# SrikarK-code/clip-dplm

Hardware: NVIDIA B200
Metric: contrastive_fwd_bwd_pairs_per_sec (higher is better)
Workload: dtype bf16

## Files before the change

clip-dplm_b200/csrc/clipnce_api.cu:

```cuda
#include <cuda.h>
#include <cuda_bf16.h>
#include <cuda_runtime.h>

#include <cmath>
#include <cstdarg>
#include <cstdio>
#include <cstdlib>
#include <cstring>
#include <mutex>
#include <set>
#include <string>
#include <utility>

#include "../../include/clipnce.h"
#include "kernels_aux.cuh"
#include "kernels_head.cuh"
#include "kernels_link.cuh"
#include "kernels_pair.cuh"
#include "kernels_pair2.cuh"
#include "kernels_simt.cuh"
#include "kernels_tc.cuh"

namespace {

thread_local std::string g_err;

int fail(int code, const char* fmt, ...) {
  char buf[512];
  va_list ap;
  va_start(ap, fmt);
  vsnprintf(buf, sizeof buf, fmt, ap);
  va_end(ap);
  g_err = buf;
  return code;
}

#define CUDA_TRY(expr)                                                                              \
  do {                                                                                              \
    cudaError_t e_ = (expr);                                                                        \
    if (e_ != cudaSuccess) return fail(CLIPNCE_ECUDA, "%s: %s", #expr, cudaGetErrorString(e_));     \
  } while (0)

// ... 927 lines not shown
  const dim3 grid((unsigned)pl.n_blk, (unsigned)n_members);
  const int64_t slab_elems = 2 * V * d;
#define FINISH_G(TI, TO)                                                                                                  \
  aux::finish_rows_group<__nv_bfloat16, TI, TO><<<grid, 256, smem, st>>>(slabs, pl.bwd_n_split, slab_elems, fg,          \
                                                                        (const __nv_bfloat16*)stack, (const TI*)stack_orig, \
                                                                        rinv, di, (TO*)d_stack, ds_part, sq_part)
  if (in_dtype == CLIPNCE_BF16 && out_dtype == CLIPNCE_BF16) FINISH_G(__nv_bfloat16, __nv_bfloat16);
  else if (in_dtype == CLIPNCE_BF16) FINISH_G(__nv_bfloat16, float);
  else if (out_dtype == CLIPNCE_BF16) FINISH_G(float, __nv_bfloat16);
  else FINISH_G(float, float);
#undef FINISH_G
  CUDA_TRY(cudaGetLastError());
  if (d_scale_sum || grad_sumsq) {
    aux::reduce_group_scalars<<<1 + n_members, 256, 0, st>>>(ds_part, sq_part, n_members, pl.n_blk, d_scale_sum, grad_sumsq);
    CUDA_TRY(cudaGetLastError());
  }
  return 0;
}

}

namespace {
struct Bwd2Plan {
  int P, Q, n_rb, n_seg, seg_steps, n_items, n_rounds, n_steps, n_half, depth, stages_a, stages_b, stages_c, smem;
  size_t off_flags, off_ring, off_dxh, off_dyh, off_part, bytes;
};

bool bwd2_device_ok() {
  if (env_int("CLIPNCE_NO_BWD2", 0) != 0) return false;
  if (allow_smem(pair2::bwd2_kernel<false>, pair::SMEM_LIMIT) || allow_smem(pair2::bwd2_kernel<true>, pair::SMEM_LIMIT)) {
    cudaGetLastError();
    return false;
  }
  static const bool ok = [] {
    cudaLaunchConfig_t cfg;
    memset(&cfg, 0, sizeof cfg);
    cfg.gridDim = dim3(2 * pair_slots());
    cfg.blockDim = dim3(pair2::THREADS);
    cfg.dynamicSmemBytes = pair::SMEM_LIMIT;
    int n = 0, n2 = 0;
    if (cudaOccupancyMaxActiveClusters(&n, pair2::bwd2_kernel<false>, &cfg) != cudaSuccess ||
        cudaOccupancyMaxActiveClusters(&n2, pair2::bwd2_kernel<true>, &cfg) != cudaSuccess) {
      cudaGetLastError();
      return false;
    }
    return n >= pair_slots() && n2 >= pair_slots();
  }();
  return ok;
}

bool bwd2_plan(int64_t n_rows, int64_t n_cols, int64_t d, int dtype, float scale, int flags, int world, Bwd2Plan* pl) {
  const int fam = tc_family(dtype, d, scale, flags);
  if (!((fam == 1 || fam == 2) && pair_eligible(d)) || (flags & CLIPNCE_FLAG_UNBOUNDED)) return false;
  if (world == 1 || world < 0 || world > pair2::MAX_WORLD) return false;
  if (world == 0 ? n_rows != n_cols : n_rows * world != n_cols) return false;
  const int64_t min_n = env_int("CLIPNCE_BWD2_MIN_N", 12288);
  if (n_rows % 128 != 0 || n_cols % 256 != 0 || n_rows * n_cols < min_n * min_n || n_cols > (1ll << 22)) return false;
  if (world >= 2 && (n_cols / world) % 256 != 0) return false;
  const int slots = pair_slots();
  if (slots < 8) return false;
  pl->n_rb = (int)(n_rows / 128);
  pl->n_steps = (int)(n_cols / 256);
  pl->n_half = (int)ceil_div(d, 256);
  const int forced_p = (int)env_int("CLIPNCE_BWD2_P", 0);
  const int forced_seg = (int)env_int("CLIPNCE_BWD2_SEG", 0);
  constexpr double r = 1.0;
  double best_t = 1e300;
  int best_p = 0, best_seg = 0;
  for (int n_seg = 1; n_seg <= 8; n_seg *= 2) {
    int ns = world >= 2 ? world : n_seg;
    if (world == 0 && forced_seg >= 1) ns = forced_seg;
    if (pl->n_steps % ns != 0) continue;
    const int seg_steps = pl->n_steps / ns;
    if (seg_steps < 8 && ns > 1 && world == 0 && forced_seg < 1) continue;
    const int64_t n_items = (int64_t)pl->n_rb * ns;
    const double slab_steps = (double)(ns - 1) * (double)n_rows * (double)d * 8.0 / 3e12 / 3.9e-6;
    const bool force = forced_p >= 1 && forced_p <= slots - 1;
    for (int Pe = force ? forced_p : slots / 2; Pe <= (force ? forced_p : slots - 2); ++Pe) {
      const int Q = slots - Pe;
      const double tp = (double)ceil_div(n_items, Pe) * ((double)seg_steps + 1.0);
      const double tc_ = (double)n_items * (double)seg_steps / ((double)Q * 2.0 * r);
      const double t = ((tp > tc_ ? tp : tc_) + slab_steps) * (world == 0 && ns > 1 ? 1.08 : 1.0);
      if (t < best_t - 1e-9) { best_t = t; best_p = Pe; best_seg = ns; }
    }
    if (world >= 2 || forced_seg >= 1) break;
  }
  if (best_p == 0) return false;
  pl->P = best_p;
  pl->Q = slots - best_p;
  pl->n_seg = best_seg;
  pl->seg_steps = pl->n_steps / best_seg;
  pl->n_items = pl->n_rb * best_seg;
  pl->n_rounds = (int)ceil_div(pl->n_items, pl->P);
  pl->depth = pair2::RING_DEPTH;
  const int nkc = (int)(d / 64);
  const int total = (pair::SMEM_LIMIT - pair2::producer_smem(nkc, 0)) / pair::STAGE_BYTES;
  if (total < 4) return false;
  auto cap = [](int v) { return v > pair2::MAXS ? pair2::MAXS : v; };
  pl->stages_b = cap(total / 2);
  pl->stages_a = cap(total - total / 2);
  pl->stages_c = cap((pair::SMEM_LIMIT - pair2::consumer_smem(0)) / pair2::C_STAGE);
  const int ps = pair2::producer_smem(nkc, pl->stages_a + pl->stages_b), cs = pair2::consumer_smem(pl->stages_c);
  pl->smem = ps > cs ? ps : cs;
  size_t off = 0;
  auto region = [&](size_t bytes) { const size_t o = off; off = (size_t)round_up((int64_t)(off + bytes), 256); return o; };
  pl->off_flags = region(sizeof(uint32_t) * 2 * (size_t)pl->n_rounds * (size_t)pl->seg_steps);
  pl->off_ring = region((size_t)pl->depth * (size_t)pl->P * 128 * 256 * 2);
  pl->off_dxh = region(sizeof(float) * (size_t)pl->n_seg * (size_t)n_rows * (size_t)d);
  pl->off_dyh = region(sizeof(float) * (size_t)n_cols * (size_t)d);
  pl->off_part = region(sizeof(float) * (size_t)ceil_div(n_rows > n_cols ? n_rows : n_cols, 8));
  pl->bytes = off;
  return true;
}

int launch_finish(const float* parts, int n_split, int64_t slab_elems, const void* xc, const void* xo, int in_dtype,
                  const float* rinv, const float* grad_scale, int64_t n, int64_t d, void* dx, int out_dtype, float* ds_part,
                  cudaStream_t st) {
  const unsigned grid = (unsigned)ceil_div(n, 8);
  const size_t smem = sizeof(float) * 8 * (size_t)d;
  const int di = (int)d;
#define FINISH3(TI, TO)                                                                                                \
  aux::finish_rows_v4<__nv_bfloat16, TI, TO><<<grid, 256, smem, st>>>(parts, n_split, slab_elems, (const __nv_bfloat16*)xc, \
                                                                      (const TI*)xo, rinv, grad_scale, n, di, (TO*)dx, ds_part)
  if (in_dtype == CLIPNCE_BF16 && out_dtype == CLIPNCE_BF16) FINISH3(__nv_bfloat16, __nv_bfloat16);
  else if (in_dtype == CLIPNCE_BF16) FINISH3(__nv_bfloat16, float);
  else if (out_dtype == CLIPNCE_BF16) FINISH3(float, __nv_bfloat16);
  else FINISH3(float, float);
#undef FINISH3
  CUDA_TRY(cudaGetLastError());
  return 0;
// ... 1 lines not shown

int bwd2_launch(const Bwd2Plan& pl, const void* x, const void* y, const float* rinv_x, const float* rinv_y, int64_t n_rows,
                int64_t n_cols, int64_t d, int64_t diag_offset, float scale, const float* scale_dev, const float* row_m,
                const float* row_w, const float* col_m, const float* col_w, float diag_w, char* ws, float* const* dy_peer,
                int world, cudaStream_t st) {
  uint32_t* flags_dev = reinterpret_cast<uint32_t*>(ws + pl.off_flags);
  const size_t n_flags = (size_t)pl.n_rounds * (size_t)pl.seg_steps;
  CUDA_TRY(cudaMemsetAsync(flags_dev, 0, sizeof(uint32_t) * 2 * n_flags, st));
  pair2::Params p;
  memset(&p, 0, sizeof p);
  p.n_rows = (int)n_rows; p.n_cols = (int)n_cols; p.d = (int)d;
  p.nkc = (int)(d / 64); p.nq2 = (int)ceil_div(d, 256); p.n_half = pl.n_half;
  p.nsbuf = p.nq2 <= 2 ? 2 : 1;
  p.n_rb = pl.n_rb; p.n_seg = pl.n_seg; p.seg_steps = pl.seg_steps; p.n_items = pl.n_items; p.n_rounds = pl.n_rounds;
  p.P = pl.P; p.Q = pl.Q; p.depth = pl.depth;
  p.stages_a = pl.stages_a; p.stages_b = pl.stages_b; p.stages_c = pl.stages_c;
  p.diag_offset = diag_offset; p.scale = scale; p.scale_dev = scale_dev; p.diag_w = diag_w;
  p.rinv_x = rinv_x; p.rinv_y = rinv_y; p.row_m = row_m; p.row_w = row_w; p.col_m = col_m; p.col_w = col_w;
  p.dx = reinterpret_cast<float*>(ws + pl.off_dxh);
  p.dy = reinterpret_cast<float*>(ws + pl.off_dyh);
  p.world = world;
  for (int s = 0; s < world; ++s) p.dy_peer[s] = dy_peer[s];
  p.ready = flags_dev; p.done = flags_dev + n_flags;
  CUtensorMap tx, ty, tyg, tg;
  int rc;
  if ((rc = make_tmap(&tx, x, d, n_rows, d, pair2::ROWS))) return rc;
  if ((rc = make_tmap(&ty, y, d, n_cols, d, 128))) return rc;
  if ((rc = make_tmap(&tyg, y, d, n_cols, d, 64))) return rc;
  if ((rc = make_tmap(&tg, ws + pl.off_ring, 256, (int64_t)pl.depth * pl.P * 128, 256, 64))) return rc;
  auto kern = tc_family(CLIPNCE_BF16, d, scale, 0) == 2 ? pair2::bwd2_kernel<true> : pair2::bwd2_kernel<false>;
  if ((rc = allow_smem(kern, pair::SMEM_LIMIT))) return rc;
  kern<<<2 * (pl.P + pl.Q), pair2::THREADS, pl.smem, st>>>(tx, ty, tyg, tg, p);
  CUDA_TRY(cudaGetLastError());
  return 0;
}
}

extern "C" {

int clipnce_backward_both_workspace_bytes(int64_t n_rows, int64_t n_cols, int64_t d, int dtype, float scale, int flags,
                                          int world, size_t* out) {
  if (!out) return fail(CLIPNCE_EINVAL, "backward_both_workspace_bytes: null pointer");
  Bwd2Plan pl;
  *out = (n_rows >= 1 && n_cols >= 1 && d >= 1 && bwd2_plan(n_rows, n_cols, d, dtype, scale, flags, world, &pl) &&
          check_device_sm100() == 0 && bwd2_device_ok()) ? pl.bytes : 0;
  return 0;
}

int clipnce_backward_both_dx(const void* x, const void* y, const float* rinv_x, const float* rinv_y, int64_t n,
                             int64_t d, float scale, const float* scale_dev, const float* row_m, const float* row_w,
                             const float* col_m, const float* col_w, float diag_w, int dtype, int flags,
                             const void* x_orig, const void* y_orig, int in_dtype, const float* grad_scale, void* dx,
                             void* dy, int out_dtype, float* d_scale_sum, void* workspace, size_t workspace_bytes,
                             void* stream) {
  if (!x || !y || !rinv_x || !rinv_y || !row_m || !row_w || !col_m || !col_w || !x_orig || !y_orig || !dx || !dy || !workspace)
    return fail(CLIPNCE_EINVAL, "backward_both_dx: null pointer");
  if ((in_dtype != CLIPNCE_BF16 && in_dtype != CLIPNCE_F32) || (out_dtype != CLIPNCE_BF16 && out_dtype != CLIPNCE_F32))
    return fail(CLIPNCE_EINVAL, "backward_both_dx: bad dtype");
  if (in_dtype == dtype && (x_orig != x || y_orig != y))
    return fail(CLIPNCE_EINVAL, "backward_both_dx: x_orig / y_orig of the compute type must be x / y themselves");
  if (!aligned16(x) || !aligned16(y) || !aligned16(workspace)) return fail(CLIPNCE_EINVAL, "backward_both_dx: operands must be 16-byte aligned");
  int rc = check_device_sm100();
  if (rc) return rc;
  Bwd2Plan pl;
  if (!bwd2_plan(n, n, d, dtype, scale, flags, 0, &pl) || !bwd2_device_ok())
    return fail(CLIPNCE_EUNSUPPORTED, "backward_both_dx: shape not served (see clipnce_backward_both_workspace_bytes)");
  if (workspace_bytes < pl.bytes) return fail(CLIPNCE_EWORKSPACE, "backward_both_dx: workspace %zu < %zu", workspace_bytes, pl.bytes);
  cudaStream_t st = as_stream(stream);
  char* ws = reinterpret_cast<char*>(workspace);
  if ((rc = bwd2_launch(pl, x, y, rinv_x, rinv_y, n, n, d, 0, scale, scale_dev, row_m, row_w, col_m, col_w, diag_w, ws, nullptr,
                        0, st)))
    return rc;
  float* ds_part = reinterpret_cast<float*>(ws + pl.off_part);
  if ((rc = launch_finish(reinterpret_cast<float*>(ws + pl.off_dxh), pl.n_seg, n * d, x, x_orig, in_dtype, rinv_x, grad_scale, n, d,
                          dx, out_dtype, d_scale_sum ? ds_part : nullptr, st)))
    return rc;
  if ((rc = launch_finish(reinterpret_cast<float*>(ws + pl.off_dyh), 1, n * d, y, y_orig, in_dtype, rinv_y, grad_scale, n, d, dy,
                          out_dtype, nullptr, st)))
    return rc;
  if (d_scale_sum) {
    aux::reduce_scalar_partials_par<<<1, 256, 0, st>>>(ds_part, (int)ceil_div(n, 8), 1.f, d_scale_sum);
    CUDA_TRY(cudaGetLastError());
  }
  return 0;
}

int clipnce_backward_both_sharded(const void* x, const void* y, const float* rinv_x, const float* rinv_y, int64_t n_rows,
                                  int64_t n_cols, int64_t d, int64_t diag_offset, float scale, const float* scale_dev,
                                  const float* row_m, const float* row_w, const float* col_m, const float* col_w,
                                  float diag_w, int dtype, int flags, const void* x_orig, int in_dtype,
                                  const float* grad_scale, void* dx, int out_dtype, float* d_scale_sum,
                                  void* const* peer_base, int world, int rank, int64_t slots_offset, void* workspace,
                                  size_t workspace_bytes, void* stream) {
  if (!x || !y || !rinv_x || !rinv_y || !row_m || !row_w || !col_m || !col_w || !x_orig || !workspace || !peer_base)
    return fail(CLIPNCE_EINVAL, "backward_both_sharded: null pointer");
  if ((in_dtype != CLIPNCE_BF16 && in_dtype != CLIPNCE_F32) || (out_dtype != CLIPNCE_BF16 && out_dtype != CLIPNCE_F32))
    return fail(CLIPNCE_EINVAL, "backward_both_sharded: bad dtype");
  if (in_dtype == dtype && x_orig != x) return fail(CLIPNCE_EINVAL, "backward_both_sharded: x_orig of the compute type must be x itself");
  if (!aligned16(x) || !aligned16(y) || !aligned16(workspace)) return fail(CLIPNCE_EINVAL, "backward_both_sharded: operands must be 16-byte aligned");
  if (world < 2 || world > pair2::MAX_WORLD || rank < 0 || rank >= world || slots_offset < 0 || slots_offset % 16 != 0)
    return fail(CLIPNCE_EINVAL, "backward_both_sharded: bad world / rank / slots_offset");
  if (diag_offset != (int64_t)rank * n_rows) return fail(CLIPNCE_EINVAL, "backward_both_sharded: diag_offset must be rank * n_rows");
  int rc = check_device_sm100();
  if (rc) return rc;
  Bwd2Plan pl;
  if (!bwd2_plan(n_rows, n_cols, d, dtype, scale, flags, world, &pl) || !bwd2_device_ok())
    return fail(CLIPNCE_EUNSUPPORTED, "backward_both_sharded: shape not served (see clipnce_backward_both_workspace_bytes)");
  if (workspace_bytes < pl.bytes) return fail(CLIPNCE_EWORKSPACE, "backward_both_sharded: workspace %zu < %zu", workspace_bytes, pl.bytes);
  cudaStream_t st = as_stream(stream);
  char* ws = reinterpret_cast<char*>(workspace);
  float* dy_peer[pair2::MAX_WORLD];
  for (int s = 0; s < world; ++s) {
    if (!peer_base[s] || !aligned16(peer_base[s])) return fail(CLIPNCE_EINVAL, "backward_both_sharded: peer buffer %d is null or unaligned", s);
    dy_peer[s] = reinterpret_cast<float*>(reinterpret_cast<char*>(peer_base[s]) + slots_offset) + (size_t)rank * (size_t)n_rows * (size_t)d;
  }
  if ((rc = bwd2_launch(pl, x, y, rinv_x, rinv_y, n_rows, n_cols, d, diag_offset, scale, scale_dev, row_m, row_w, col_m, col_w,
                        diag_w, ws, dy_peer, world, st)))
    return rc;
  if (!dx) return 0;
  float* ds_part = reinterpret_cast<float*>(ws + pl.off_part);
  if ((rc = launch_finish(reinterpret_cast<float*>(ws + pl.off_dxh), pl.n_seg, n_rows * d, x, x_orig, in_dtype, rinv_x, grad_scale,
                          n_rows, d, dx, out_dtype, d_scale_sum ? ds_part : nullptr, st)))
    return rc;
  if (d_scale_sum) {
    aux::reduce_scalar_partials_par<<<1, 256, 0, st>>>(ds_part, (int)ceil_div(n_rows, 8), 1.f, d_scale_sum);
    CUDA_TRY(cudaGetLastError());
  }
  return 0;
}
// ... 355 lines not shown
```

clip-dplm_b200/csrc/kernels_pair2.cuh:

```cuda
#pragma once
#include "kernels_pair.cuh"

namespace pair2 {

using pair::LOG2E;
using pair::STAGE_BYTES;
using pair::STEP_J;
using pair::TMEM_COLS;

constexpr int THREADS = 416;
constexpr int STORE_WARP = 12;
constexpr int EPI_WARPS = 8;
constexpr int ROWS = 64;
constexpr int X_CHUNK = ROWS * 128;
constexpr int G_BYTES = 4 * 8192;
constexpr int SMALL = 10240;
constexpr int C_STAGE = 32768;
constexpr int MAXS = 6;
constexpr int RING_DEPTH = 16;
constexpr int MAX_WORLD = 16;

constexpr int B_FULL_A = 0, B_EMPTY_A = MAXS, B_FULL_B = 2 * MAXS, B_EMPTY_B = 3 * MAXS, B_XFULL = 4 * MAXS,
              B_XEMPTY = B_XFULL + 1, B_SFULL = B_XEMPTY + 1, B_SEMPTY = B_SFULL + 2, B_GFULL = B_SEMPTY + 2,
              B_GEMPTY = B_GFULL + 4, B_ACCFULL = B_GEMPTY + 4, B_ACCEMPTY = B_ACCFULL + 2, B_GSFULL = B_ACCEMPTY + 2,
// ... 2 lines not shown

struct Params {
  int n_rows, n_cols, d;
  int nsbuf;
  int nkc, nq2, n_half;
  int n_rb, n_seg, seg_steps, n_items, n_rounds;
  int P, Q, depth;
  int stages_a, stages_b, stages_c;
  long long diag_offset;
  float scale, diag_w;
  const float* scale_dev;
  const float* rinv_x;
  const float* rinv_y;
  const float* row_m;
  const float* row_w;
  const float* col_m;
  const float* col_w;
  float* dx;
  float* dy;
  float* dy_peer[MAX_WORLD];
  int world;
  uint32_t* ready;
  uint32_t* done;
};

__host__ __device__ constexpr int producer_smem(int nkc, int stages) {
  return nkc * X_CHUNK + G_BYTES + stages * STAGE_BYTES + SMALL;
}
constexpr int FLUSH_BYTES = EPI_WARPS * 4096;
__host__ __device__ constexpr int consumer_smem(int stages) { return stages * C_STAGE + FLUSH_BYTES + SMALL; }
__device__ __forceinline__ float4 ld_shared_v4(uint32_t addr) {
  float4 v;
  asm volatile("ld.shared.v4.f32 {%0, %1, %2, %3}, [%4];" : "=f"(v.x), "=f"(v.y), "=f"(v.z), "=f"(v.w) : "r"(addr) : "memory");
  return v;
}

__device__ __forceinline__ void publish(uint32_t* flag) {
  ptx::fence_proxy_async_all();
  ptx::red_release_gpu_add(flag, 1u);
}

struct Sub {
  int seg, p_lo, p_hi, rb_lo;
  bool first, last;
};
__device__ __forceinline__ int round_items(const Params& p, int r) { return min(p.P, p.n_items - r * p.P); }
// ... 557 lines not shown
```

Measured before the change: 4.394 million.

## Add three-role backward kernel splitting producer, dX partner, and dY consumer

Introduces a new bwd3 kernel in which separate CTA pairs handle the logits/gradient producer, the dX accumulation partner, and the dY consumer, with 256-row blocks per item. It becomes the default for d up to 512. The planner is reworked to split SMs among the three roles, and the co-residency check is generalised per kernel and smem size. The intent is to balance tensor-core work across more specialized roles and to free producer shared memory for deeper pipelines. This adds a large new kernel and more inter-CTA flag synchronisation.

```diff
diff --git a/clip-dplm_b200/csrc/clipnce_api.cu b/clip-dplm_b200/csrc/clipnce_api.cu
--- a/clip-dplm_b200/csrc/clipnce_api.cu
+++ b/clip-dplm_b200/csrc/clipnce_api.cu
@@ -10,6 +10,7 @@
 #include <mutex>
 #include <set>
 #include <string>
+#include <tuple>
 #include <utility>
 
 #include "../../include/clipnce.h"
@@ -18,6 +19,7 @@
 #include "kernels_link.cuh"
 #include "kernels_pair.cuh"
 #include "kernels_pair2.cuh"
+#include "kernels_pair3.cuh"
 #include "kernels_simt.cuh"
 #include "kernels_tc.cuh"
 
@@ -991,31 +993,47 @@
 
 namespace {
 struct Bwd2Plan {
+  int roles;
+  int fam;
   int P, Q, n_rb, n_seg, seg_steps, n_items, n_rounds, n_steps, n_half, depth, stages_a, stages_b, stages_c, smem;
   size_t off_flags, off_ring, off_dxh, off_dyh, off_part, bytes;
 };
 
-bool bwd2_device_ok() {
-  if (env_int("CLIPNCE_NO_BWD2", 0) != 0) return false;
-  if (allow_smem(pair2::bwd2_kernel<false>, pair::SMEM_LIMIT) || allow_smem(pair2::bwd2_kernel<true>, pair::SMEM_LIMIT)) {
+std::set<std::tuple<const void*, int, int>> g_coresident;
+
+template <typename Kernel>
+bool coresident(Kernel* kern, int smem) {
+  int dev = 0;
+  if (allow_smem(kern, pair::SMEM_LIMIT) || cudaGetDevice(&dev) != cudaSuccess) {
     cudaGetLastError();
     return false;
   }
-  static const bool ok = [] {
-    cudaLaunchConfig_t cfg;
-    memset(&cfg, 0, sizeof cfg);
-    cfg.gridDim = dim3(2 * pair_slots());
-    cfg.blockDim = dim3(pair2::THREADS);
-    cfg.dynamicSmemBytes = pair::SMEM_LIMIT;
-    int n = 0, n2 = 0;
-    if (cudaOccupancyMaxActiveClusters(&n, pair2::bwd2_kernel<false>, &cfg) != cudaSuccess ||
-        cudaOccupancyMaxActiveClusters(&n2, pair2::bwd2_kernel<true>, &cfg) != cudaSuccess) {
-      cudaGetLastError();
-      return false;
-    }
-    return n >= pair_slots() && n2 >= pair_slots();
-  }();
-  return ok;
+  const auto key = std::make_tuple(reinterpret_cast<const void*>(kern), smem, dev);
+  {
+    std::lock_guard<std::mutex> lk(g_mu);
+    if (g_coresident.count(key)) return true;
+  }
+  cudaLaunchConfig_t cfg;
+  memset(&cfg, 0, sizeof cfg);
+  cfg.gridDim = dim3(2 * pair_slots());
+  cfg.blockDim = dim3(pair2::THREADS);
+  cfg.dynamicSmemBytes = smem;
+  int n = 0;
+  if (cudaOccupancyMaxActiveClusters(&n, kern, &cfg) != cudaSuccess) {
+    cudaGetLastError();
+    return false;
+  }
+  if (n < pair_slots()) return false;
+  std::lock_guard<std::mutex> lk(g_mu);
+  g_coresident.insert(key);
+  return true;
+}
+
+bool bwd2_device_ok(const Bwd2Plan& pl) {
+  if (env_int("CLIPNCE_NO_BWD2", 0) != 0) return false;
+  if (pl.roles == 3)
+    return pl.fam == 2 ? coresident(pair3::bwd3_kernel<true>, pl.smem) : coresident(pair3::bwd3_kernel<false>, pl.smem);
+  return pl.fam == 2 ? coresident(pair2::bwd2_kernel<true>, pl.smem) : coresident(pair2::bwd2_kernel<false>, pl.smem);
 }
 
 bool bwd2_plan(int64_t n_rows, int64_t n_cols, int64_t d, int dtype, float scale, int flags, int world, Bwd2Plan* pl) {
@@ -1028,12 +1046,17 @@
   if (world >= 2 && (n_cols / world) % 256 != 0) return false;
   const int slots = pair_slots();
   if (slots < 8) return false;
-  pl->n_rb = (int)(n_rows / 128);
+  pl->roles = d <= pair3::MAX_D && env_int("CLIPNCE_BWD2_ROLES", 3) != 2 ? 3 : 2;
+  pl->fam = tc_family(CLIPNCE_BF16, d, scale, 0) == 2 ? 2 : 1;
+  const int rb_rows = pl->roles == 3 ? 256 : 128;
+  pl->n_rb = (int)(n_rows / rb_rows);
   pl->n_steps = (int)(n_cols / 256);
   pl->n_half = (int)ceil_div(d, 256);
-  const int forced_p = (int)env_int("CLIPNCE_BWD2_P", 0);
+  const int p_max = pl->roles == 3 ? (slots - 1) / 2 : slots - 1;
+  const int forced_p = (int)std::min<int64_t>(env_int("CLIPNCE_BWD2_P", 0), p_max);
   const int forced_seg = (int)env_int("CLIPNCE_BWD2_SEG", 0);
-  constexpr double r = 1.0;
+  const double r = pl->roles == 3 ? 1.0 : 2.0;
+  const int p_lo = pl->roles == 3 ? 1 : slots / 2, p_hi = pl->roles == 3 ? p_max : slots - 2;
   double best_t = 1e300;
   int best_p = 0, best_seg = 0;
   for (int n_seg = 1; n_seg <= 8; n_seg *= 2) {
@@ -1044,11 +1067,11 @@
     if (seg_steps < 8 && ns > 1 && world == 0 && forced_seg < 1) continue;
     const int64_t n_items = (int64_t)pl->n_rb * ns;
     const double slab_steps = (double)(ns - 1) * (double)n_rows * (double)d * 8.0 / 3e12 / 3.9e-6;
-    const bool force = forced_p >= 1 && forced_p <= slots - 1;
-    for (int Pe = force ? forced_p : slots / 2; Pe <= (force ? forced_p : slots - 2); ++Pe) {
-      const int Q = slots - Pe;
+    const bool force = forced_p >= 1;
+    for (int Pe = force ? forced_p : p_lo; Pe <= (force ? forced_p : p_hi); ++Pe) {
+      const int Q = slots - (pl->roles == 3 ? 2 * Pe : Pe);
       const double tp = (double)ceil_div(n_items, Pe) * ((double)seg_steps + 1.0);
-      const double tc_ = (double)n_items * (double)seg_steps / ((double)Q * 2.0 * r);
+      const double tc_ = (double)n_items * (double)seg_steps / ((double)Q * r);
       const double t = ((tp > tc_ ? tp : tc_) + slab_steps) * (world == 0 && ns > 1 ? 1.08 : 1.0);
       if (t < best_t - 1e-9) { best_t = t; best_p = Pe; best_seg = ns; }
     }
@@ -1056,25 +1079,32 @@
   }
   if (best_p == 0) return false;
   pl->P = best_p;
-  pl->Q = slots - best_p;
+  pl->Q = slots - (pl->roles == 3 ? 2 * best_p : best_p);
   pl->n_seg = best_seg;
   pl->seg_steps = pl->n_steps / best_seg;
   pl->n_items = pl->n_rb * best_seg;
   pl->n_rounds = (int)ceil_div(pl->n_items, pl->P);
   pl->depth = pair2::RING_DEPTH;
   const int nkc = (int)(d / 64);
-  const int total = (pair::SMEM_LIMIT - pair2::producer_smem(nkc, 0)) / pair::STAGE_BYTES;
-  if (total < 4) return false;
   auto cap = [](int v) { return v > pair2::MAXS ? pair2::MAXS : v; };
-  pl->stages_b = cap(total / 2);
-  pl->stages_a = cap(total - total / 2);
   pl->stages_c = cap((pair::SMEM_LIMIT - pair2::consumer_smem(0)) / pair2::C_STAGE);
-  const int ps = pair2::producer_smem(nkc, pl->stages_a + pl->stages_b), cs = pair2::consumer_smem(pl->stages_c);
-  pl->smem = ps > cs ? ps : cs;
+  const int cs = pair2::consumer_smem(pl->stages_c);
+  if (pl->roles == 3) {
+    const int nq2 = (int)ceil_div(d, 256);
+    pl->stages_a = cap((pair::SMEM_LIMIT - pair3::producer_smem(nkc, 0)) / pair::STAGE_BYTES);
+    pl->stages_b = cap((pair::SMEM_LIMIT - pair3::partner_smem(nq2, 0)) / pair3::partner_stage(nq2));
+    pl->smem = std::max(std::max(pair3::producer_smem(nkc, pl->stages_a), pair3::partner_smem(nq2, pl->stages_b)), cs);
+  } else {
+    const int total = (pair::SMEM_LIMIT - pair2::producer_smem(nkc, 0)) / pair::STAGE_BYTES;
+    if (total < 4) return false;
+    pl->stages_b = cap(total / 2);
+    pl->stages_a = cap(total - total / 2);
+    pl->smem = std::max(pair2::producer_smem(nkc, pl->stages_a + pl->stages_b), cs);
+  }
   size_t off = 0;
   auto region = [&](size_t bytes) { const size_t o = off; off = (size_t)round_up((int64_t)(off + bytes), 256); return o; };
   pl->off_flags = region(sizeof(uint32_t) * 2 * (size_t)pl->n_rounds * (size_t)pl->seg_steps);
-  pl->off_ring = region((size_t)pl->depth * (size_t)pl->P * 128 * 256 * 2);
+  pl->off_ring = region((size_t)pl->depth * (size_t)pl->P * rb_rows * 256 * 2);
   pl->off_dxh = region(sizeof(float) * (size_t)pl->n_seg * (size_t)n_rows * (size_t)d);
   pl->off_dyh = region(sizeof(float) * (size_t)n_cols * (size_t)d);
   pl->off_part = region(sizeof(float) * (size_t)ceil_div(n_rows > n_cols ? n_rows : n_cols, 8));
@@ -1122,15 +1152,28 @@
   p.world = world;
   for (int s = 0; s < world; ++s) p.dy_peer[s] = dy_peer[s];
   p.ready = flags_dev; p.done = flags_dev + n_flags;
+  p.ring = ws + pl.off_ring;
   CUtensorMap tx, ty, tyg, tg;
   int rc;
-  if ((rc = make_tmap(&tx, x, d, n_rows, d, pair2::ROWS))) return rc;
+  const int rb_rows = pl.roles == 3 ? 256 : 128;
+  const int64_t ring_rows = (int64_t)pl.depth * pl.P * rb_rows;
   if ((rc = make_tmap(&ty, y, d, n_cols, d, 128))) return rc;
   if ((rc = make_tmap(&tyg, y, d, n_cols, d, 64))) return rc;
-  if ((rc = make_tmap(&tg, ws + pl.off_ring, 256, (int64_t)pl.depth * pl.P * 128, 256, 64))) return rc;
-  auto kern = tc_family(CLIPNCE_BF16, d, scale, 0) == 2 ? pair2::bwd2_kernel<true> : pair2::bwd2_kernel<false>;
-  if ((rc = allow_smem(kern, pair::SMEM_LIMIT))) return rc;
-  kern<<<2 * (pl.P + pl.Q), pair2::THREADS, pl.smem, st>>>(tx, ty, tyg, tg, p);
+  if ((rc = make_tmap(&tg, ws + pl.off_ring, 256, ring_rows, 256, 64))) return rc;
+  if (pl.roles == 3) {
+    CUtensorMap tx64, tg128;
+    if ((rc = make_tmap(&tx, x, d, n_rows, d, pair3::ROWS))) return rc;
+    if ((rc = make_tmap(&tx64, x, d, n_rows, d, 64))) return rc;
+    if ((rc = make_tmap(&tg128, ws + pl.off_ring, 256, ring_rows, 256, 128))) return rc;
+    auto kern = pl.fam == 2 ? pair3::bwd3_kernel<true> : pair3::bwd3_kernel<false>;
+    if ((rc = allow_smem(kern, pair::SMEM_LIMIT))) return rc;
+    kern<<<2 * (2 * pl.P + pl.Q), pair2::THREADS, pl.smem, st>>>(tx, tx64, ty, tyg, tg, tg128, p);
+  } else {
+    if ((rc = make_tmap(&tx, x, d, n_rows, d, pair2::ROWS))) return rc;
+    auto kern = pl.fam == 2 ? pair2::bwd2_kernel<true> : pair2::bwd2_kernel<false>;
+    if ((rc = allow_smem(kern, pair::SMEM_LIMIT))) return rc;
+    kern<<<2 * (pl.P + pl.Q), pair2::THREADS, pl.smem, st>>>(tx, ty, tyg, tg, p);
+  }
   CUDA_TRY(cudaGetLastError());
   return 0;
 }
@@ -1143,7 +1186,7 @@
   if (!out) return fail(CLIPNCE_EINVAL, "backward_both_workspace_bytes: null pointer");
   Bwd2Plan pl;
   *out = (n_rows >= 1 && n_cols >= 1 && d >= 1 && bwd2_plan(n_rows, n_cols, d, dtype, scale, flags, world, &pl) &&
-          check_device_sm100() == 0 && bwd2_device_ok()) ? pl.bytes : 0;
+          check_device_sm100() == 0 && bwd2_device_ok(pl)) ? pl.bytes : 0;
   return 0;
 }
 
@@ -1163,7 +1206,7 @@
   int rc = check_device_sm100();
   if (rc) return rc;
   Bwd2Plan pl;
-  if (!bwd2_plan(n, n, d, dtype, scale, flags, 0, &pl) || !bwd2_device_ok())
+  if (!bwd2_plan(n, n, d, dtype, scale, flags, 0, &pl) || !bwd2_device_ok(pl))
     return fail(CLIPNCE_EUNSUPPORTED, "backward_both_dx: shape not served (see clipnce_backward_both_workspace_bytes)");
   if (workspace_bytes < pl.bytes) return fail(CLIPNCE_EWORKSPACE, "backward_both_dx: workspace %zu < %zu", workspace_bytes, pl.bytes);
   cudaStream_t st = as_stream(stream);
@@ -1204,7 +1247,7 @@
   int rc = check_device_sm100();
   if (rc) return rc;
   Bwd2Plan pl;
-  if (!bwd2_plan(n_rows, n_cols, d, dtype, scale, flags, world, &pl) || !bwd2_device_ok())
+  if (!bwd2_plan(n_rows, n_cols, d, dtype, scale, flags, world, &pl) || !bwd2_device_ok(pl))
     return fail(CLIPNCE_EUNSUPPORTED, "backward_both_sharded: shape not served (see clipnce_backward_both_workspace_bytes)");
   if (workspace_bytes < pl.bytes) return fail(CLIPNCE_EWORKSPACE, "backward_both_sharded: workspace %zu < %zu", workspace_bytes, pl.bytes);
   cudaStream_t st = as_stream(stream);
diff --git a/clip-dplm_b200/csrc/kernels_pair2.cuh b/clip-dplm_b200/csrc/kernels_pair2.cuh
--- a/clip-dplm_b200/csrc/kernels_pair2.cuh
+++ b/clip-dplm_b200/csrc/kernels_pair2.cuh
@@ -48,6 +48,7 @@
   int world;
   uint32_t* ready;
   uint32_t* done;
+  void* ring;
 };
 
 __host__ __device__ constexpr int producer_smem(int nkc, int stages) {
diff --git a/clip-dplm_b200/csrc/kernels_pair3.cuh b/clip-dplm_b200/csrc/kernels_pair3.cuh
--- /dev/null
+++ b/clip-dplm_b200/csrc/kernels_pair3.cuh
@@ -0,0 +1,609 @@
+#pragma once
+#include "kernels_pair2.cuh"
+
+namespace pair3 {
+
+using pair::LOG2E;
+using pair::STAGE_BYTES;
+using pair::STEP_J;
+using pair::TMEM_COLS;
+using pair2::C_STAGE;
+using pair2::EPI_WARPS;
+using pair2::FLUSH_BYTES;
+using pair2::MAXS;
+using pair2::Params;
+using pair2::SMALL;
+using pair2::STORE_WARP;
+using pair2::Sub;
+using pair2::THREADS;
+
+constexpr int ROWS = 128;
+constexpr int X_CHUNK = ROWS * 128;
+constexpr int SBUF_COLS = 256;
+constexpr int MAX_D = 512;
+
+constexpr int B_FULL = 0, B_EMPTY = MAXS, B_XFULL = 2 * MAXS, B_XEMPTY = B_XFULL + 1, B_SFULL = B_XEMPTY + 1,
+              B_SEMPTY = B_SFULL + 2, B_ACCFULL = B_SEMPTY + 2, B_ACCEMPTY = B_ACCFULL + 2, B_SLOTFREE = B_ACCEMPTY + 2,
+              B_GW = B_SLOTFREE + 1, B_STEPDONE = B_GW + 1, B_STEPACK = B_STEPDONE + 2, B_COUNT = B_STEPACK + 2;
+static_assert(B_COUNT * 8 <= 1000, "barrier block");
+
+constexpr int G_SCRATCH = 2048;
+__host__ __device__ constexpr int producer_smem(int nkc, int stages) {
+  return nkc * X_CHUNK + stages * STAGE_BYTES + EPI_WARPS * G_SCRATCH + SMALL;
+}
+__host__ __device__ constexpr int partner_stage(int nq2) { return STAGE_BYTES * (1 + nq2); }
+__host__ __device__ constexpr int partner_smem(int nq2, int stages) { return stages * partner_stage(nq2) + SMALL; }
+static_assert(producer_smem(MAX_D / 64, 4) <= pair::SMEM_LIMIT, "producer: resident X + 4 Y stages + scratch at d = 512");
+static_assert(partner_smem(MAX_D / 256, 3) <= pair::SMEM_LIMIT, "dX partner: 3 stages at d = 512");
+static_assert(pair2::consumer_smem(3) <= pair::SMEM_LIMIT, "dY consumer: 3 stages");
+static_assert(2 * SBUF_COLS <= TMEM_COLS && MAX_D <= TMEM_COLS && 2 * 256 <= TMEM_COLS, "TMEM: every role fits 512 columns");
+
+__device__ __forceinline__ void st_global_v4_hint(void* p, uint32_t a, uint32_t b, uint32_t c, uint32_t d, uint64_t pol) {
+  asm volatile("st.global.L2::cache_hint.v4.b32 [%0], {%1, %2, %3, %4}, %5;" ::"l"(p), "r"(a), "r"(b), "r"(c), "r"(d), "l"(pol)
+               : "memory");
+}
+__device__ __forceinline__ uint32_t done_target(const Params& p, int r) {
+  return (uint32_t)(pair2::round_subs(p, r) * p.n_half + pair2::round_items(p, r));
+}
+
+template <bool TWO_EXP>
+__global__ void __cluster_dims__(2, 1, 1) __launch_bounds__(THREADS, 1)
+bwd3_kernel(const __grid_constant__ CUtensorMap tmap_x,
+            const __grid_constant__ CUtensorMap tmap_x64,
+            const __grid_constant__ CUtensorMap tmap_y,
+            const __grid_constant__ CUtensorMap tmap_yg,
+            const __grid_constant__ CUtensorMap tmap_g,
+            const __grid_constant__ CUtensorMap tmap_g128,
+            const Params p) {
+  extern __shared__ __align__(1024) uint8_t smem[];
+  const uint32_t base = ptx::smem_u32(smem);
+  if ((base & 1023u) != 0) __trap();
+  const uint32_t rank = ptx::cluster_ctarank();
+  const bool leader = rank == 0;
+  const int warp = threadIdx.x >> 5;
+  const int lane = threadIdx.x & 31;
+  const int pair_id = blockIdx.x >> 1;
+  const int role = pair_id < p.P ? 0 : pair_id < 2 * p.P ? 1 : 2;
+  const int nq2 = (p.d + 255) >> 8;
+
+  const int body = max(max(producer_smem(p.nkc, p.stages_a), partner_smem(nq2, p.stages_b)), pair2::consumer_smem(p.stages_c)) - SMALL;
+  const uint32_t bars = base + body;
+  auto bar = [&](int i) -> uint32_t { return bars + 8u * i; };
+  volatile uint32_t* tmem_ptr_smem = reinterpret_cast<volatile uint32_t*>(smem + body + 1016);
+  float* const colv = reinterpret_cast<float*>(smem + body + 1024);
+
+  const float sc = p.scale_dev != nullptr ? __ldg(p.scale_dev) : p.scale;
+  const float k2 = sc * LOG2E;
+
+  if (warp == 0 && lane == 0) {
+    ptx::prefetch_tmap(&tmap_x);
+    ptx::prefetch_tmap(&tmap_x64);
+    ptx::prefetch_tmap(&tmap_y);
+    ptx::prefetch_tmap(&tmap_yg);
+    ptx::prefetch_tmap(&tmap_g);
+    ptx::prefetch_tmap(&tmap_g128);
+  }
+  if (warp == 1 && lane == 0) {
+    for (int s = 0; s < MAXS; ++s) {
+      ptx::mbar_init(bar(B_FULL + s), 1);
+      ptx::mbar_init(bar(B_EMPTY + s), 1);
+    }
+    ptx::mbar_init(bar(B_XFULL), 1);
+    ptx::mbar_init(bar(B_XEMPTY), 1);
+    for (int b = 0; b < 2; ++b) {
+      ptx::mbar_init(bar(B_SFULL + b), 1);
+      ptx::mbar_init(bar(B_SEMPTY + b), 2 * EPI_WARPS);
+      ptx::mbar_init(bar(B_ACCFULL + b), 1);
+      ptx::mbar_init(bar(B_ACCEMPTY + b), 2 * EPI_WARPS);
+      ptx::mbar_init(bar(B_STEPDONE + b), 1);
+      ptx::mbar_init(bar(B_STEPACK + b), 1);
+    }
+    ptx::mbar_init(bar(B_SLOTFREE), 1);
+    ptx::mbar_init(bar(B_GW), EPI_WARPS);
+    ptx::fence_mbar_init();
+  }
+  if (warp == 2) ptx::tmem_alloc_pair(ptx::smem_u32(const_cast<uint32_t*>(tmem_ptr_smem)), TMEM_COLS);
+  ptx::tc_fence_before();
+  __syncthreads();
+  ptx::cluster_sync();
+  ptx::tc_fence_after();
+  const uint32_t tmem_base = *tmem_ptr_smem;
+
+  const uint32_t desc_hi_k = static_cast<uint32_t>(ptx::smem_desc_k_sw128(0) >> 32);
+  const uint32_t desc_hi_mn = static_cast<uint32_t>(ptx::smem_desc_mn_sw128(0, 8192) >> 32);
+  auto desc_lo = [&](uint32_t addr, uint32_t lbo16) -> uint32_t { return ((addr & 0x3FFFFu) >> 4) | (lbo16 << 16); };
+  auto mk = [&](uint32_t hi, uint32_t lo) -> uint64_t { return (static_cast<uint64_t>(hi) << 32) | lo; };
+
+  if (role == 0) {
+    const uint32_t x_smem = base;
+    const uint32_t ring_a = x_smem + p.nkc * X_CHUNK;
+
+    if (warp == 0) {
+      if (ptx::elect_one()) {
+        int stage = 0;
+        uint32_t phase = 0;
+        for (int r = 0; r < p.n_rounds; ++r) {
+          const int item = r * p.P + pair_id;
+          if (item >= p.n_items) break;
+          const int i0 = (item % p.n_rb) * (2 * ROWS) + (int)rank * ROWS;
+          const int t0 = (item / p.n_rb) * p.seg_steps;
+          ptx::mbar_wait(bar(B_XEMPTY), (r & 1) ^ 1u);
+          if (leader) ptx::mbar_arrive_expect_tx(bar(B_XFULL), 2 * p.nkc * X_CHUNK);
+          for (int kc = 0; kc < p.nkc; ++kc) ptx::tma_load_2d_pair(x_smem + kc * X_CHUNK, &tmap_x, bar(B_XFULL), kc * 64, i0);
+          for (int t = t0; t < t0 + p.seg_steps; ++t) {
+            for (int g = 0; g < p.nkc; ++g) {
+              ptx::mbar_wait(bar(B_EMPTY + stage), phase ^ 1u);
+              if (leader) ptx::mbar_arrive_expect_tx(bar(B_FULL + stage), 2 * STAGE_BYTES);
+              ptx::tma_load_2d_pair(ring_a + stage * STAGE_BYTES, &tmap_y, bar(B_FULL + stage), g * 64, t * STEP_J + (int)rank * 128);
+              if (++stage == p.stages_a) { stage = 0; phase ^= 1u; }
+            }
+          }
+        }
+      }
+      __syncwarp();
+    } else if (warp == 1) {
+      if (leader && ptx::elect_one()) {
+        constexpr uint32_t idesc_s = ptx::idesc_bf16_f32_major(2 * ROWS, STEP_J, 0, 0);
+        const uint32_t x_lo0 = desc_lo(x_smem, 1), a_lo0 = desc_lo(ring_a, 1);
+        int stage = 0;
+        uint32_t phase = 0, ready = 0, gs = 0;
+        for (int r = 0; r < p.n_rounds; ++r) {
+          if (r * p.P + pair_id >= p.n_items) break;
+          ptx::mbar_wait(bar(B_XFULL), r & 1);
+          for (int t = 0; t < p.seg_steps; ++t, ++gs) {
+            const int sb = gs & 1;
+            ptx::mbar_wait(bar(B_SEMPTY + sb), ((gs >> 1) & 1) ^ 1u);
+            const uint32_t d_tmem = tmem_base + sb * SBUF_COLS;
+            for (int g = 0; g < p.nkc; ++g) {
+              if (!ready) ptx::mbar_wait(bar(B_FULL + stage), phase);
+              ptx::tc_fence_after();
+              int ns = stage + 1;
+              uint32_t np = phase;
+              if (ns == p.stages_a) { ns = 0; np ^= 1u; }
+              ready = ptx::mma_box_pair(d_tmem, mk(desc_hi_k, x_lo0 + g * (X_CHUNK >> 4)),
+                                        mk(desc_hi_k, a_lo0 + stage * (STAGE_BYTES >> 4)), 2, 2, idesc_s, g != 0,
+                                        bar(B_FULL + ns), np);
+              ptx::mma_commit_pair(bar(B_EMPTY + stage));
+              if (g == p.nkc - 1) ptx::mma_commit_pair(bar(B_SFULL + sb));
+              stage = ns;
+              phase = np;
+            }
+          }
+          ptx::mma_commit_pair(bar(B_XEMPTY));
+        }
+      }
+      __syncwarp();
+    } else if (warp == STORE_WARP) {
+      if (ptx::elect_one()) {
+        for (int r = 0; r < p.n_rounds; ++r) {
+          if (r * p.P + pair_id >= p.n_items) break;
+          for (int t = 0; t < p.seg_steps; ++t) {
+            const uint32_t g = (uint32_t)r * (uint32_t)p.seg_steps + (uint32_t)t;
+            if (g >= (uint32_t)p.depth) {
+              const uint32_t go = g - (uint32_t)p.depth;
+              ptx::spin_until_ge(p.done + go, done_target(p, (int)(go / (uint32_t)p.seg_steps)));
+            }
+            ptx::mbar_arrive(bar(B_SLOTFREE));
+            ptx::mbar_wait(bar(B_GW), g & 1u);
+            pair2::publish(p.ready + g);
+          }
+        }
+      }
+      __syncwarp();
+    } else if (warp >= 4 && warp < 4 + EPI_WARPS) {
+      const int e = warp - 4;
+      const int q = warp & 3;
+      const int h = e >> 2;
+      const int i_local = 32 * q + lane;
+      const int te = threadIdx.x - 128;
+      const uint32_t t_lane = tmem_base + (static_cast<uint32_t>(q * 32) << 16);
+      const uint32_t sempty_leader = ptx::mapa(bar(B_SEMPTY), 0);
+      const uint64_t keep = ptx::l2_policy_evict_last();
+      __nv_bfloat16* const ring = reinterpret_cast<__nv_bfloat16*>(p.ring);
+      const uint32_t scratch = base + p.nkc * X_CHUNK + p.stages_a * STAGE_BYTES + e * G_SCRATCH;
+      const int rsub = lane >> 2, ch = lane & 3;
+      uint32_t gs = 0;
+
+      for (int r = 0; r < p.n_rounds; ++r) {
+        const int item = r * p.P + pair_id;
+        if (item >= p.n_items) break;
+        const int seg = item / p.n_rb;
+        const int t0 = seg * p.seg_steps;
+        const int i_glob = (item % p.n_rb) * (2 * ROWS) + (int)rank * ROWS + i_local;
+        const float rx = p.rinv_x[i_glob];
+        const float u = TWO_EXP ? 0.f : p.row_w[i_glob] * pair::ex2((sc - p.row_m[i_glob]) * LOG2E);
+        const float rm2 = TWO_EXP ? p.row_m[i_glob] * LOG2E : 0.f;
+        const float rw = TWO_EXP ? p.row_w[i_glob] : 0.f;
+        const long long dcol = (long long)i_glob + p.diag_offset;
+        float cw_n, cm_n, ry_n;
+        {
+          const long long jn = (long long)t0 * STEP_J + te;
+          cw_n = p.col_w[jn]; cm_n = p.col_m[jn]; ry_n = p.rinv_y[jn];
+        }
+
+        for (int t = t0; t < t0 + p.seg_steps; ++t, ++gs) {
+          const uint32_t g = (uint32_t)r * (uint32_t)p.seg_steps + (uint32_t)(t - t0);
+          const int sb = gs & 1;
+          float* const cv = colv + (gs & 1) * 1024;
+          cv[te] = ry_n * k2;
+          cv[256 + te] = (TWO_EXP ? cw_n : cw_n * pair::ex2((sc - cm_n) * LOG2E)) * ry_n;
+          cv[512 + te] = ry_n;
+          if (TWO_EXP) cv[768 + te] = cw_n > 0.f ? cm_n * LOG2E : 0.f;
+          if (t + 1 < t0 + p.seg_steps) {
+            const long long jn = (long long)(t + 1) * STEP_J + te;
+            cw_n = p.col_w[jn]; cm_n = p.col_m[jn]; ry_n = p.rinv_y[jn];
+          }
+          pair::named_bar_sync(1, EPI_WARPS * 32);
+          __nv_bfloat16* const wrow =
+              ring + ((long long)((int)(g % (uint32_t)p.depth) * p.P + pair_id) * (2 * ROWS) + (int)rank * ROWS + 32 * q) * STEP_J;
+
+          ptx::mbar_wait(bar(B_SFULL + sb), (gs >> 1) & 1);
+          ptx::tc_fence_after();
+#pragma unroll 1
+          for (int b = 0; b < 2; ++b) {
+            const int col0 = 128 * h + 64 * b;
+            const long long dl = dcol - ((long long)t * STEP_J + col0);
+            const bool has_diag = dl >= 0 && dl < 64;
+            uint32_t pk[32];
+#pragma unroll
+            for (int c = 0; c < 2; ++c) {
+              uint32_t rr[32];
+              ptx::tmem_ld_32x32b_x32(t_lane + sb * SBUF_COLS + col0 + 32 * c, rr);
+              ptx::tmem_ld_wait();
+              if (b == 1 && c == 1) {
+                ptx::tc_fence_before();
+                __syncwarp();
+                if (lane == 0) ptx::mbar_arrive_cluster(sempty_leader + 8u * sb);
+              }
+              const float* const cjp = cv + col0 + 32 * c;
+#pragma unroll
+              for (int x4 = 0; x4 < 8; ++x4) {
+                const float4 cj4 = *reinterpret_cast<const float4*>(cjp + 4 * x4);
+                const float4 vr4 = *reinterpret_cast<const float4*>(cjp + 256 + 4 * x4);
+                const float4 ry4 = *reinterpret_cast<const float4*>(cjp + 512 + 4 * x4);
+                const float cjv[4] = {cj4.x, cj4.y, cj4.z, cj4.w};
+                const float vrv[4] = {vr4.x, vr4.y, vr4.z, vr4.w};
+                const float ryv[4] = {ry4.x, ry4.y, ry4.z, ry4.w};
+                float gv[4];
+                if constexpr (TWO_EXP) {
+                  const float4 cm4 = *reinterpret_cast<const float4*>(cjp + 768 + 4 * x4);
+                  const float cmv[4] = {cm4.x, cm4.y, cm4.z, cm4.w};
+#pragma unroll
+                  for (int xx = 0; xx < 4; ++xx) {
+                    const float y = __uint_as_float(rr[4 * x4 + xx]) * rx;
+                    const float er = pair::ex2(fmaf(y, cjv[xx], -rm2)) * rw;
+                    const float ec = pair::ex2(fmaf(y, cjv[xx], -cmv[xx]));
+                    gv[xx] = rx * fmaf(er, ryv[xx], ec * vrv[xx]);
+                  }
+                } else {
+#pragma unroll
+                  for (int xx = 0; xx < 4; ++xx) {
+                    const float y = __uint_as_float(rr[4 * x4 + xx]) * rx;
+                    const float ev = pair::ex2(fmaf(y, cjv[xx], -k2)) * rx;
+                    gv[xx] = ev * fmaf(u, ryv[xx], vrv[xx]);
+                  }
+                }
+                if (has_diag) {
+#pragma unroll
+                  for (int xx = 0; xx < 4; ++xx)
+                    if (dl == 32 * c + 4 * x4 + xx) gv[xx] -= p.diag_w * rx * ryv[xx];
+                }
+                const __nv_bfloat162 p0 = __floats2bfloat162_rn(gv[0], gv[1]);
+                const __nv_bfloat162 p1 = __floats2bfloat162_rn(gv[2], gv[3]);
+                pk[16 * c + 2 * x4] = *reinterpret_cast<const uint32_t*>(&p0);
+                pk[16 * c + 2 * x4 + 1] = *reinterpret_cast<const uint32_t*>(&p1);
+              }
+            }
+            if (b == 0) ptx::mbar_wait(bar(B_SLOTFREE), gs & 1u);
+#pragma unroll
+            for (int c = 0; c < 2; ++c) {
+#pragma unroll
+              for (int k = 0; k < 4; ++k)
+                pair::st_shared_v4(scratch + lane * 64 + ((static_cast<uint32_t>(k) ^ ((lane >> 1) & 3)) << 4), pk[16 * c + 4 * k],
+                                   pk[16 * c + 4 * k + 1], pk[16 * c + 4 * k + 2], pk[16 * c + 4 * k + 3]);
+              __syncwarp();
+#pragma unroll
+              for (int i = 0; i < 4; ++i) {
+                const int row = 8 * i + rsub;
+                uint32_t v0, v1, v2, v3;
+                asm volatile("ld.shared.v4.b32 {%0, %1, %2, %3}, [%4];"
+                             : "=r"(v0), "=r"(v1), "=r"(v2), "=r"(v3)
+                             : "r"(scratch + row * 64 + ((static_cast<uint32_t>(ch) ^ ((row >> 1) & 3)) << 4))
+                             : "memory");
+                st_global_v4_hint(wrow + (long long)row * STEP_J + col0 + 32 * c + 8 * ch, v0, v1, v2, v3, keep);
+              }
+              __syncwarp();
+            }
+          }
+          __syncwarp();
+          if (lane == 0) ptx::mbar_arrive(bar(B_GW));
+        }
+      }
+    }
+  } else if (role == 1) {
+    const int pp = pair_id - p.P;
+    const int pstage = partner_stage(nq2);
+
+    if (warp == 0) {
+      if (ptx::elect_one()) {
+        int stage = 0;
+        uint32_t phase = 0;
+        const uint64_t keep = ptx::l2_policy_evict_last();
+        for (int r = 0; r < p.n_rounds; ++r) {
+          const int item = r * p.P + pp;
+          if (item >= p.n_items) break;
+          const int t0 = (item / p.n_rb) * p.seg_steps;
+          const uint32_t want = 2u * (uint32_t)pair2::round_items(p, r);
+          for (int tau = 0; tau < p.seg_steps; ++tau) {
+            const uint32_t g = (uint32_t)r * (uint32_t)p.seg_steps + (uint32_t)tau;
+            const int grow = ((int)(g % (uint32_t)p.depth) * p.P + pp) * (2 * ROWS) + (int)rank * ROWS;
+            const int t = t0 + tau;
+            ptx::spin_until_ge(p.ready + g, want);
+            ptx::fence_proxy_async_all();
+            for (int kc = 0; kc < 4; ++kc) {
+              ptx::mbar_wait(bar(B_EMPTY + stage), phase ^ 1u);
+              const uint32_t st = base + stage * pstage;
+              int bytes = STAGE_BYTES;
+              for (int q = 0; q < nq2; ++q) bytes += (min(256, p.d - 256 * q) >> 7) * 8192;
+              if (leader) ptx::mbar_arrive_expect_tx(bar(B_FULL + stage), 2 * bytes);
+              ptx::tma_load_2d_pair_hint(st, &tmap_g128, bar(B_FULL + stage), 64 * kc, grow, keep);
+              for (int q = 0; q < nq2; ++q) {
+                const int half = min(256, p.d - 256 * q) >> 1;
+                for (int gi = 0; gi < (half >> 6); ++gi)
+                  ptx::tma_load_2d_pair(st + STAGE_BYTES * (1 + q) + gi * 8192, &tmap_yg, bar(B_FULL + stage),
+                                        256 * q + half * (int)rank + 64 * gi, t * STEP_J + 64 * kc);
+              }
+              if (++stage == p.stages_b) { stage = 0; phase ^= 1u; }
+            }
+          }
+        }
+      }
+      __syncwarp();
+    } else if (warp == 1) {
+      if (leader && ptx::elect_one()) {
+        int stage = 0;
+        uint32_t phase = 0, ready = 0, gs = 0;
+        for (int r = 0; r < p.n_rounds; ++r) {
+          if (r * p.P + pp >= p.n_items) break;
+          ptx::mbar_wait(bar(B_ACCEMPTY), (r & 1) ^ 1u);
+          ptx::tc_fence_after();
+          for (int tau = 0; tau < p.seg_steps; ++tau, ++gs) {
+            for (int kc = 0; kc < 4; ++kc) {
+              if (!ready) ptx::mbar_wait(bar(B_FULL + stage), phase);
+              ptx::tc_fence_after();
+              int ns = stage + 1;
+              uint32_t np = phase;
+              if (ns == p.stages_b) { ns = 0; np ^= 1u; }
+              const uint32_t st = base + stage * pstage;
+              for (int q = 0; q < nq2; ++q) {
+                const uint32_t idesc = ptx::idesc_bf16_f32_major(2 * ROWS, min(256, p.d - 256 * q), 0, 1);
+                const bool last = q == nq2 - 1;
+                const uint32_t rdy = ptx::mma_box_pair(tmem_base + 256 * q, mk(desc_hi_k, desc_lo(st, 1)),
+                                                       mk(desc_hi_mn, desc_lo(st + STAGE_BYTES * (1 + q), 8192 >> 4)), 2,
+                                                       2048 >> 4, idesc, (tau | kc) != 0,
+                                                       last ? bar(B_FULL + ns) : bar(B_FULL + stage), last ? np : phase);
+                if (last) ready = rdy;
+              }
+              ptx::mma_commit_pair(bar(B_EMPTY + stage));
+              stage = ns;
+              phase = np;
+            }
+            const int b = gs & 1;
+            ptx::mbar_wait(bar(B_STEPACK + b), ((gs >> 1) & 1) ^ 1u);
+            ptx::mma_commit_pair(bar(B_STEPDONE + b));
+          }
+          ptx::mma_commit_pair(bar(B_ACCFULL));
+        }
+      }
+      __syncwarp();
+    } else if (warp == 3) {
+      if (leader && ptx::elect_one()) {
+        uint32_t gs = 0;
+        for (int r = 0; r < p.n_rounds; ++r) {
+          if (r * p.P + pp >= p.n_items) break;
+          for (int tau = 0; tau < p.seg_steps; ++tau, ++gs) {
+            const int b = gs & 1;
+            ptx::mbar_wait(bar(B_STEPDONE + b), (gs >> 1) & 1);
+            ptx::red_release_gpu_add(p.done + ((uint32_t)r * (uint32_t)p.seg_steps + (uint32_t)tau), 1u);
+            ptx::mbar_arrive(bar(B_STEPACK + b));
+          }
+        }
+      }
+      __syncwarp();
+    } else if (warp >= 4 && warp < 4 + EPI_WARPS) {
+      const int q = warp & 3;
+      const int h = (warp - 4) >> 2;
+      const uint32_t t_lane = tmem_base + (static_cast<uint32_t>(q * 32) << 16);
+      const uint32_t accempty_leader = ptx::mapa(bar(B_ACCEMPTY), 0);
+      for (int r = 0; r < p.n_rounds; ++r) {
+        const int item = r * p.P + pp;
+        if (item >= p.n_items) break;
+        const int seg = item / p.n_rb;
+        const int i_glob = (item % p.n_rb) * (2 * ROWS) + (int)rank * ROWS + 32 * q + lane;
+        const float osc = sc / p.rinv_x[i_glob];
+        float* const dst = p.dx + (long long)seg * p.n_rows * p.d + (long long)i_glob * p.d;
+        ptx::mbar_wait(bar(B_ACCFULL), r & 1);
+        ptx::tc_fence_after();
+        for (int c = h; c < (p.d >> 5); c += 2) {
+          uint32_t rr[32];
+          ptx::tmem_ld_32x32b_x32(t_lane + 32 * c, rr);
+          ptx::tmem_ld_wait();
+#pragma unroll
+          for (int x4 = 0; x4 < 8; ++x4)
+            *reinterpret_cast<float4*>(dst + 32 * c + 4 * x4) =
+                make_float4(__uint_as_float(rr[4 * x4]) * osc, __uint_as_float(rr[4 * x4 + 1]) * osc,
+                            __uint_as_float(rr[4 * x4 + 2]) * osc, __uint_as_float(rr[4 * x4 + 3]) * osc);
+        }
+        ptx::tc_fence_before();
+        __syncwarp();
+        if (lane == 0) ptx::mbar_arrive_cluster(accempty_leader);
+      }
+    }
+  } else {
+    const int cidx = pair_id - 2 * p.P;
+    const uint32_t ring_c = base;
+
+    if (warp == 0) {
+      if (ptx::elect_one()) {
+        int stage = 0;
+        uint32_t phase = 0;
+        const uint64_t keep = ptx::l2_policy_evict_last();
+        for (int r = 0; r < p.n_rounds; ++r) {
+          const int pw = pair2::round_items(p, r);
+          const int nsub = pair2::round_subs(p, r);
+          for (int tau = 0; tau < p.seg_steps; ++tau) {
+            const uint32_t g = (uint32_t)r * (uint32_t)p.seg_steps + (uint32_t)tau;
+            const int slot = (int)(g % (uint32_t)p.depth);
+            bool step_ready = false;
+            for (int k = 0; k < nsub; ++k) {
+              const Sub sub = pair2::round_sub(p, r, k);
+              const int t = sub.seg * p.seg_steps + tau;
+              for (int hh = 0; hh < p.n_half; ++hh) {
+                if ((t * p.n_half + hh) % p.Q != cidx) continue;
+                if (!step_ready) {
+                  ptx::spin_until_ge(p.ready + g, 2u * (uint32_t)pw);
+                  ptx::fence_proxy_async_all();
+                  step_ready = true;
+                }
+                const int wq = min(256, p.d - 256 * hh);
+                const int ngr = wq >> 7;
+                for (int pq = sub.p_lo; pq < sub.p_hi; ++pq) {
+                  for (int kb = 0; kb < 4; ++kb) {
+                    ptx::mbar_wait(bar(B_EMPTY + stage), phase ^ 1u);
+                    if (leader) ptx::mbar_arrive_expect_tx(bar(B_FULL + stage), 2 * (2 + ngr) * 8192);
+                    const uint32_t st = ring_c + stage * C_STAGE;
+                    const int grow = (slot * p.P + pq) * (2 * ROWS) + 64 * kb;
+                    const int xrow = (sub.rb_lo + pq - sub.p_lo) * (2 * ROWS) + 64 * kb;
+                    for (int gi = 0; gi < 2; ++gi)
+                      ptx::tma_load_2d_pair_hint(st + gi * 8192, &tmap_g, bar(B_FULL + stage), 128 * (int)rank + 64 * gi, grow, keep);
+                    for (int gi = 0; gi < ngr; ++gi)
+                      ptx::tma_load_2d_pair(st + 16384 + gi * 8192, &tmap_x64, bar(B_FULL + stage),
+                                            256 * hh + (wq >> 1) * (int)rank + 64 * gi, xrow);
+                    if (++stage == p.stages_c) { stage = 0; phase ^= 1u; }
+                  }
+                }
+              }
+            }
+          }
+        }
+      }
+      __syncwarp();
+    } else if (warp == 1) {
+      if (leader && ptx::elect_one()) {
+        const uint32_t a_lo0 = desc_lo(ring_c, 8192 >> 4), b_lo0 = desc_lo(ring_c + 16384, 8192 >> 4);
+        int stage = 0;
+        uint32_t phase = 0, ready = 0, nt = 0;
+        for (int r = 0; r < p.n_rounds; ++r) {
+          const int nsub = pair2::round_subs(p, r);
+          for (int tau = 0; tau < p.seg_steps; ++tau) {
+            for (int k = 0; k < nsub; ++k) {
+              const Sub sub = pair2::round_sub(p, r, k);
+              const int t = sub.seg * p.seg_steps + tau;
+              for (int hh = 0; hh < p.n_half; ++hh) {
+                if ((t * p.n_half + hh) % p.Q != cidx) continue;
+                const int buf = nt & 1;
+                ptx::mbar_wait(bar(B_ACCEMPTY + buf), ((nt >> 1) & 1) ^ 1u);
+                ptx::tc_fence_after();
+                const int wq = min(256, p.d - 256 * hh);
+                const uint32_t idesc = ptx::idesc_bf16_f32_major(256, wq, 1, 1);
+                const uint32_t d_tmem = tmem_base + buf * 256;
+                const int nk = 4 * (sub.p_hi - sub.p_lo);
+                for (int kk = 0; kk < nk; ++kk) {
+                  if (!ready) ptx::mbar_wait(bar(B_FULL + stage), phase);
+                  ptx::tc_fence_after();
+                  int ns = stage + 1;
+                  uint32_t np = phase;
+                  if (ns == p.stages_c) { ns = 0; np ^= 1u; }
+                  ready = ptx::mma_box_pair(d_tmem, mk(desc_hi_mn, a_lo0 + stage * (C_STAGE >> 4)),
+                                            mk(desc_hi_mn, b_lo0 + stage * (C_STAGE >> 4)), 2048 >> 4, 2048 >> 4, idesc,
+                                            kk != 0, bar(B_FULL + ns), np);
+                  ptx::mma_commit_pair(bar(B_EMPTY + stage));
+                  stage = ns;
+                  phase = np;
+                }
+                ptx::mma_commit_pair(bar(B_ACCFULL + buf));
+                ++nt;
+              }
+            }
+          }
+        }
+      }
+      __syncwarp();
+    } else if (warp >= 4 && warp < 4 + EPI_WARPS) {
+      const int q = warp & 3;
+      const int hcol = (warp - 4) >> 2;
+      const uint32_t t_lane = tmem_base + (static_cast<uint32_t>(q * 32) << 16);
+      const uint32_t accempty_leader = ptx::mapa(bar(B_ACCEMPTY), 0);
+      const uint32_t scratch = ring_c + p.stages_c * C_STAGE + (warp - 4) * 4096;
+      uint32_t nt = 0;
+      for (int r = 0; r < p.n_rounds; ++r) {
+        const int nsub = pair2::round_subs(p, r);
+        for (int tau = 0; tau < p.seg_steps; ++tau) {
+          for (int k = 0; k < nsub; ++k) {
+            const Sub sub = pair2::round_sub(p, r, k);
+            const int t = sub.seg * p.seg_steps + tau;
+            for (int hh = 0; hh < p.n_half; ++hh) {
+              if ((t * p.n_half + hh) % p.Q != cidx) continue;
+              const int buf = nt & 1;
+              const long long j = (long long)t * STEP_J + (int)rank * 128 + 32 * q + lane;
+              const float osc = sc / p.rinv_y[j];
+              ptx::mbar_wait(bar(B_ACCFULL + buf), (nt >> 1) & 1);
+              ptx::tc_fence_after();
+              if (leader && warp == 4 && lane == 0)
+                ptx::red_release_gpu_add(p.done + ((uint32_t)r * (uint32_t)p.seg_steps + (uint32_t)tau), 1u);
+              const int wq = min(256, p.d - 256 * hh);
+              const int wh = wq >> 1;
+              const long long col0 = 256 * hh + hcol * wh;
+              const long long j0 = j - lane;
+              const bool remote = sub.last && p.world > 0;
+              float* const obase = remote ? p.dy_peer[sub.seg] + (j0 - (long long)sub.seg * p.seg_steps * STEP_J) * p.d + col0
+                                          : p.dy + j0 * p.d + col0;
+              const float* const lbase = p.dy + j0 * p.d + col0;
+              const int rsub = lane >> 3, ch = lane & 7;
+              for (int c = 0; c < (wh >> 5); ++c) {
+                uint32_t rr[32];
+                ptx::tmem_ld_32x32b_x32(t_lane + buf * 256 + hcol * wh + 32 * c, rr);
+                ptx::tmem_ld_wait();
+#pragma unroll
+                for (int k4 = 0; k4 < 8; ++k4)
+                  pair::st_shared_v4(scratch + lane * 128 + ((static_cast<uint32_t>(k4) ^ (lane & 7)) << 4),
+                                     __float_as_uint(__uint_as_float(rr[4 * k4]) * osc), __float_as_uint(__uint_as_float(rr[4 * k4 + 1]) * osc),
+                                     __float_as_uint(__uint_as_float(rr[4 * k4 + 2]) * osc), __float_as_uint(__uint_as_float(rr[4 * k4 + 3]) * osc));
+                __syncwarp();
+                float4 v[8];
+#pragma unroll
+                for (int i = 0; i < 8; ++i) {
+                  const int row = 4 * i + rsub;
+                  v[i] = pair2::ld_shared_v4(scratch + row * 128 + ((static_cast<uint32_t>(ch) ^ (row & 7)) << 4));
+                }
+                if (!sub.first) {
+                  float4 old[8];
+#pragma unroll
+                  for (int i = 0; i < 8; ++i)
+                    old[i] = *reinterpret_cast<const float4*>(lbase + (long long)(4 * i + rsub) * p.d + 32 * c + 4 * ch);
+#pragma unroll
+                  for (int i = 0; i < 8; ++i) { v[i].x += old[i].x; v[i].y += old[i].y; v[i].z += old[i].z; v[i].w += old[i].w; }
+                }
+#pragma unroll
+                for (int i = 0; i < 8; ++i)
+                  *reinterpret_cast<float4*>(obase + (long long)(4 * i + rsub) * p.d + 32 * c + 4 * ch) = v[i];
+                __syncwarp();
+              }
+              ptx::tc_fence_before();
+              __syncwarp();
+              if (lane == 0) ptx::mbar_arrive_cluster(accempty_leader + 8u * buf);
+              ++nt;
+            }
+          }
+        }
+      }
+    }
+  }
+
+  ptx::tc_fence_before();
+  __syncthreads();
+  ptx::cluster_sync();
+  if (warp == 2) ptx::tmem_dealloc_pair(tmem_base, TMEM_COLS);
+}
+
+}
```

New measurement: 3.575 million, median of 6. -18.6%, worse.
